# Ulixes-8/Motion-Planning-and-Control-for-Dual-Manipulator-Robot

Measured on AMD Instinct MI355X. Metric: grasp-pose IK solves/sec (Nextage dual-arm) at 1/2/4/8 MI355X, higher is better.
Workload: dtype f64

## Files before the change

motion-planning-and-control-for-dual-manipulator-robot_amd/csrc/ikg_device.hpp:

```cpp
#pragma once

#ifndef __HIPCC_RTC__
#include <hip/hip_runtime.h>
#endif
#include <stdint.h>

#include <type_traits>

#define IKG_HD __host__ __device__

#ifndef IKG_ABL
#define IKG_ABL 0
#endif
#ifndef IKG_THETA
#define IKG_THETA 0
#endif
#ifndef IKG_TAYLOR_MUL
#define IKG_TAYLOR_MUL 1
#endif
#ifndef IKG_LOG6_SERIES
#define IKG_LOG6_SERIES 1
#endif
#ifndef IKG_LANE_LIMITS
#define IKG_LANE_LIMITS 1
// ... 77 lines not shown
  static constexpr bool zero_t(int k, int i) { return (ZMASK >> (3 * k + i)) & 1; }
  static constexpr int zmask = ZMASK;
  static constexpr bool fold_hand = axis(7) != kAxRuntime && axis(7) == axis(6);
};
using SpecGeneric = Spec<kPatternGeneric, true, false>;
using SpecGenericWrist = Spec<kPatternGeneric, true, true>;
constexpr int kPatternNextage = 2 | (2 << 2) | (1 << 4) | (1 << 6) | (0 << 8) | (1 << 10) | (2 << 12) | (2 << 14);
constexpr int kZeroNextage = (3 << 3) | (1 << 6) | (2 << 9) | (6 << 12) | (3 << 15);
using SpecNextage = Spec<kPatternNextage, false, true, kZeroNextage>;

template <typename T>
struct KParams {
  T eps;
  T dt;
  T lambda;
  int32_t max_iters;
  T eps2;
};

typedef float v2f __attribute__((ext_vector_type(2)));
typedef int v2i __attribute__((ext_vector_type(2)));

template <typename T>
struct LaneT {
  using E = T;
  using M = bool;
  static constexpr bool packed = false;
};
template <>
struct LaneT<v2f> {
  using E = float;
  using M = v2i;
  static constexpr bool packed = true;
};
template <typename T>
constexpr bool is_f64 = std::is_same<typename LaneT<T>::E, double>::value;
template <typename T>
constexpr bool is_packed = LaneT<T>::packed;

IKG_HD inline bool any_of(bool m) { return m; }
IKG_HD inline bool any_of(v2i m) { return m.x != 0 || m.y != 0; }
IKG_HD inline bool all_of(bool m) { return m; }
IKG_HD inline bool all_of(v2i m) { return m.x != 0 && m.y != 0; }
#ifndef IKG_UNIFORM
#define IKG_UNIFORM 1
#endif
template <typename T>
IKG_HD inline bool wave_any(bool b) {
#if defined(__HIP_DEVICE_COMPILE__) && IKG_UNIFORM
  if constexpr (!LaneT<T>::packed) return __builtin_amdgcn_ballot_w64(b) != 0;
#endif
  return b;
}
IKG_HD inline bool mnot(bool m) { return !m; }
IKG_HD inline v2i mnot(v2i m) { return m == 0; }
IKG_HD inline bool mor(bool a, bool b) { return a || b; }
IKG_HD inline v2i mor(v2i a, v2i b) { return a | b; }
template <typename T, typename M>
IKG_HD inline T vsel(M m, T a, T b) {
  if constexpr (LaneT<T>::packed)
    return T{m.x ? a.x : b.x, m.y ? a.y : b.y};
  else
    return m ? a : b;
}

template <typename T, typename E>
IKG_HD inline T armc(bool right, E left_v, E right_v) {
  if constexpr (is_packed<T>)
    return T{left_v, right_v};
  else
    return right ? right_v : left_v;
}

using ::atan2;
using ::atan2f;
using ::fabs;
using ::fmax;
using ::fmin;
using ::sqrt;
IKG_HD inline v2f fmax(v2f a, v2f b) { return v2f{::fmaxf(a.x, b.x), ::fmaxf(a.y, b.y)}; }
IKG_HD inline v2f fmin(v2f a, v2f b) { return v2f{::fminf(a.x, b.x), ::fminf(a.y, b.y)}; }
IKG_HD inline v2f fabs(v2f a) { return v2f{::fabsf(a.x), ::fabsf(a.y)}; }
IKG_HD inline v2f sqrt(v2f a) { return v2f{::sqrtf(a.x), ::sqrtf(a.y)}; }
IKG_HD inline v2f atan2(v2f y, v2f x) { return v2f{::atan2f(y.x, x.x), ::atan2f(y.y, x.y)}; }
IKG_HD inline v2f atan2f(v2f y, v2f x) { return atan2(y, x); }

#ifndef IKG_CW_SINCOS
#define IKG_CW_SINCOS 1
#endif
#ifndef IKG_CW_SINCOS_PACKED
#define IKG_CW_SINCOS_PACKED 0
#endif
template <typename T>
IKG_HD inline void cw_poly(T r, T& sr, T& cr) {
  const T r2 = r * r;
  T sp, cp;
  if constexpr (std::is_same<T, double>::value) {
    sp = T(-1.0 / 1307674368000.0);
    sp = fma(sp, r2, T(1.0 / 6227020800.0));
    sp = fma(sp, r2, T(-1.0 / 39916800.0));
    sp = fma(sp, r2, T(1.0 / 362880.0));
    sp = fma(sp, r2, T(-1.0 / 5040.0));
    sp = fma(sp, r2, T(1.0 / 120.0));
    sp = fma(sp, r2, T(-1.0 / 6.0));
    cp = T(1.0 / 20922789888000.0);
    cp = fma(cp, r2, T(-1.0 / 87178291200.0));
// ... 343 lines not shown
  T th, st, ct;
};
template <typename T>
struct ThetaInc;
template <>
struct ThetaInc<double> {
  static constexpr double kInc = 0.05;
  IKG_HD static inline double atan_small(double r) {
    const double r2 = r * r;
    return r + r * r2 * (-1.0 / 3 + r2 * (1.0 / 5 + r2 * (-1.0 / 7 + r2 * (1.0 / 9 + r2 * (-1.0 / 11)))));
  }
  static constexpr double kIncAsin = 0.035;
  IKG_HD static inline double asin_small(double y) {
    const double y2 = y * y;
    return y + y * y2 * (1.0 / 6 + y2 * (3.0 / 40 + y2 * (5.0 / 112 + y2 * (35.0 / 1152))));
  }
};
template <>
struct ThetaInc<float> {
  static constexpr float kInc = 0.05f;
  IKG_HD static inline float atan_small(float r) {
    const float r2 = r * r;
    return r + r * r2 * (-1.0f / 3 + r2 * (1.0f / 5 + r2 * (-1.0f / 7)));
  }
  static constexpr float kIncAsin = 0.035f;
  IKG_HD static inline float asin_small(float y) {
    const float y2 = y * y;
    return y + y * y2 * (1.0f / 6 + y2 * (3.0f / 40));
  }
};

#ifndef IKG_FAST_ATAN2
#define IKG_FAST_ATAN2 1
#endif
template <typename T>
IKG_HD inline T atan2_upper(T y, T x) {
  const T ax = fabs(x);
  const T mn = fmin(ax, y), mx = fmax(ax, y);
  const T a = fdiv<T>(mn, fmax(mx, T(1e-30f)));
  const T t = a * a;
  T u = T(0.0026226534973829985f);
  u = u * t + T(-0.015134125016629696f);
  u = u * t + T(0.0411243662238121f);
  u = u * t + T(-0.07366912066936493f);
  u = u * t + T(0.1057402640581131f);
  u = u * t + T(-0.1418599784374237f);
  u = u * t + T(0.19990399479866028f);
  u = u * t + T(-0.3333298861980438f);
  T r = a + (a * t) * u;
  r = vsel<T>(y > ax, T(1.57079637f) - r, r);
  return vsel<T>(x < T(0), T(3.14159274f) - r, r);
}

template <typename T>
IKG_HD inline void log6_iter(const T* R, const T* p, T* e, ThetaTrack<T>* tk = nullptr, bool resync = true) {
  using M = typename LaneT<T>::M;
  const T pi = T(Prec<T>::kPi);
  const T tr = R[0] + R[4] + R[8];
  const T sx = R[7] - R[5], sy = R[2] - R[6], sz = R[3] - R[1];
  const T ct = (tr - T(1)) * T(0.5);
  const T st = fsqrt_unit(sx * sx + sy * sy + sz * sz) * T(0.5);
  T theta = T(0);
  if constexpr (is_f64<T>) {
    bool exact = true;
    if (tk && !resync) {
      const T y = st * tk->ct - ct * tk->st;
      const T x = ct * tk->ct + st * tk->st;
#if IKG_THETA_ASIN
      exact = !(fabs(y) <= ThetaInc<T>::kIncAsin && x > T(0));
      theta = tk->th + ThetaInc<T>::asin_small(y);
#else
      exact = !(fabs(y) <= ThetaInc<T>::kInc * x);
      theta = tk->th + ThetaInc<T>::atan_small(fdiv<T>(y, fmax(x, T(1e-30))));
#endif
    }
    if (wave_any<T>(exact)) {
#if IKG_THETA == 1
      const T th_x = atan2(st, ct);
#else
      const T th_x = acos(fmin(fmax(ct, T(-1)), T(1)));
#endif
      theta = exact ? th_x : theta;
    }
    if (tk) {
      tk->th = theta;
      tk->st = st;
      tk->ct = ct;
    }
  } else {
#if IKG_FAST_ATAN2
    theta = atan2_upper(st, ct);
#else
    theta = atan2f(st, ct);
#endif
  }
  const T t2 = theta * theta;
  const T tiny = is_f64<T> ? T(1e-300) : T(1e-30f);
  const M above = theta > T(Prec<T>::kPrec3);
  const M below = theta < T(Prec<T>::kPrec3);
  const T q = frcp<T>(fmax(t2 * st, tiny));
  const T inv_t2 = st * q;
  T f;
  if constexpr (is_f64<T>)
    f = vsel<T>(above, theta * t2 * q, T(1));
  else
    f = vsel<T>(above, theta * t2 * q, T(1) + t2 * (T(1.f / 6) + t2 * T(7.f / 360)));
  const T hf = f * T(0.5);
  T w[3] = {hf * sx, hf * sy, hf * sz};
  T alpha = hf * (T(1) + ct);
  const M near_pi = theta >= pi - T(1e-2);
  if (wave_any<T>(any_of(near_pi))) {
    const T beta = fdiv<T>(t2, T(1) - ct);
    const T t0 = (R[0] - ct) * beta, t1 = (R[4] - ct) * beta, tt = (R[8] - ct) * beta;
    const T wp0 = vsel<T>(R[7] > R[5], T(1), T(-1)) * vsel<T>(t0 > T(0), sqrt(t0), T(0));
    const T wp1 = vsel<T>(R[2] > R[6], T(1), T(-1)) * vsel<T>(t1 > T(0), sqrt(t1), T(0));
    const T wp2 = vsel<T>(R[3] > R[1], T(1), T(-1)) * vsel<T>(tt > T(0), sqrt(tt), T(0));
    w[0] = vsel<T>(near_pi, wp0, w[0]);
    w[1] = vsel<T>(near_pi, wp1, w[1]);
    w[2] = vsel<T>(near_pi, wp2, w[2]);
    alpha = vsel<T>(near_pi, fdiv<T>(theta * st, T(2) * (T(1) - ct)), alpha);
  }
  T beta;
  if constexpr (is_f64<T>) {
#if IKG_LOG6_SERIES
#if IKG_TAYLOR_MUL
    const T as = T(1) - t2 * T(1.0 / 12) - (t2 * t2) * T(1.0 / 720);
    const T bs = T(1.0 / 12) + t2 * T(1.0 / 720);
#else
    const T as = T(1) - t2 / T(12) - t2 * t2 / T(720);
    const T bs = T(1) / T(12) + t2 / T(720);
#endif
    beta = vsel<T>(below, bs, (T(1) - alpha) * inv_t2);
    alpha = vsel<T>(below, as, alpha);
#else
    (void)below;
    beta = (T(1) - alpha) * inv_t2;
#endif
  } else {
    const T as = T(1) - t2 * (T(1.f / 12) + t2 * (T(1.f / 720) + t2 * T(1.f / 30240)));
    const T bs = T(1.f / 12) + t2 * (T(1.f / 720) + t2 * (T(1.f / 30240) + t2 * T(1.f / 1209600)));
    beta = vsel<T>(below, bs, (T(1) - alpha) * inv_t2);
    alpha = vsel<T>(below, as, alpha);
  }
  const T wp = w[0] * p[0] + w[1] * p[1] + w[2] * p[2];
  const T bwp = beta * wp;
  e[0] = alpha * p[0] - T(0.5) * (w[1] * p[2] - w[2] * p[1]) + bwp * w[0];
  e[1] = alpha * p[1] - T(0.5) * (w[2] * p[0] - w[0] * p[2]) + bwp * w[1];
  e[2] = alpha * p[2] - T(0.5) * (w[0] * p[1] - w[1] * p[0]) + bwp * w[2];
  e[3] = w[0];
  e[4] = w[1];
  e[5] = w[2];
}

template <typename T>
struct Trig;
#ifndef IKG_RESYNC64
#define IKG_RESYNC64 128
#endif
#ifndef IKG_GENERIC_MED
#define IKG_GENERIC_MED 2
#endif
template <>
struct Trig<double> {
  static constexpr double kIncMax = 0.025;
// ... 187 lines not shown
  }
  T ht[3], d[3];
  if constexpr (FOLD) {
#pragma unroll
    for (int i = 0; i < 3; ++i) ht[i] = armc<T>(right, m->hand_tH[0][i], m->hand_tH[1][i]);
    matvec3(R, ht, d);
#pragma unroll
    for (int i = 0; i < 3; ++i) th[i] = t[i] + d[i];
#pragma unroll
    for (int i = 0; i < 9; ++i) Rh[i] = R[i];
  } else {
#pragma unroll
    for (int i = 0; i < 3; ++i) ht[i] = armc<T>(right, m->hand_t[0][i], m->hand_t[1][i]);
    matvec3(R, ht, d);
#pragma unroll
    for (int i = 0; i < 3; ++i) th[i] = t[i] + d[i];
    constexpr int HA = SP::axis(7);
    if constexpr (HA != kAxRuntime) {
#pragma unroll
      for (int i = 0; i < 9; ++i) Rh[i] = R[i];
      rotate_axis(Rh, HA, armc<T>(right, m->hand_sc[0][0], m->hand_sc[1][0]),
                  armc<T>(right, m->hand_sc[0][1], m->hand_sc[1][1]));
    } else {
      T hR[9];
#pragma unroll
      for (int i = 0; i < 9; ++i) hR[i] = armc<T>(right, m->hand_R[0][i], m->hand_R[1][i]);
      matmul3(R, hR, Rh);
    }
  }
}

template <typename T, class SP>
IKG_HD inline void fk_arm_world(const KModel<typename LaneT<T>::E>* __restrict__ m, int arm, const T* sn, const T* cs, T* Rh, T* th) {
  T Rc[9], tc[3];
  root_frame<T, SP>(m, sn[0], cs[0], Rc, tc);
  fk_arm<T, SP, false>(m, arm, Rc, tc, sn, cs, Rh, th, nullptr, nullptr);
}

template <typename T>
IKG_HD inline void pose_error(const T* Rh, const T* th, const T* RT, const T* tT, T* e) {
  T Rm[9], d[3], pm[3];
  matmul3_tn(Rh, RT, Rm);
#pragma unroll
  for (int i = 0; i < 3; ++i) d[i] = tT[i] - th[i];
  matvec3_t(Rh, d, pm);
  if constexpr (IKG_ABL & 2) {
    e[0] = pm[0]; e[1] = pm[1]; e[2] = pm[2];
    e[3] = T(0.5) * (Rm[7] - Rm[5]); e[4] = T(0.5) * (Rm[2] - Rm[6]); e[5] = T(0.5) * (Rm[3] - Rm[1]);
  } else {
    log6(Rm, pm, e);
  }
}

template <typename T>
IKG_HD inline void pose_error_aligned(const T* Rh, const T* th, const T* RT, const T* tT, T* e,
                                      ThetaTrack<T>* tk = nullptr, bool resync = true) {
  T Rw[9], d[3];
  matmul3_nt(RT, Rh, Rw);
#pragma unroll
  for (int i = 0; i < 3; ++i) d[i] = tT[i] - th[i];
  if constexpr (IKG_ABL & 2) {
    e[0] = d[0]; e[1] = d[1]; e[2] = d[2];
    e[3] = T(0.5) * (Rw[7] - Rw[5]); e[4] = T(0.5) * (Rw[2] - Rw[6]); e[5] = T(0.5) * (Rw[3] - Rw[1]);
  } else {
    log6_iter(Rw, d, e, tk, resync);
  }
}

template <typename T>
IKG_HD inline void qr_solve6(T (&A)[6][8], T* x0, T* x1, bool* near_singular = nullptr, T tau = T(0)) {
#pragma unroll
  for (int k = 0; k < 5; ++k) {
    T n2 = T(0);
#pragma unroll
    for (int i = k; i < 6; ++i) n2 += A[i][k] * A[i][k];
    const T nrm = sqrt(n2);
    const T akk = A[k][k];
    const T alpha = akk >= T(0) ? -nrm : nrm;
    const T vk = akk - alpha;
    const T vtv = T(2) * nrm * (nrm + fabs(akk));
    const T scale = vtv > T(0) ? T(2) / vtv : T(0);
#pragma unroll
    for (int j = k + 1; j < 8; ++j) {
      T tau = vk * A[k][j];
#pragma unroll
      for (int i = k + 1; i < 6; ++i) tau += A[i][k] * A[i][j];
      const T f = tau * scale;
      A[k][j] -= f * vk;
#pragma unroll
      for (int i = k + 1; i < 6; ++i) A[i][j] -= f * A[i][k];
    }
    A[k][k] = alpha;
  }
  T dmax = T(0);
#pragma unroll
  for (int k = 0; k < 6; ++k) dmax = fmax(dmax, fabs(A[k][k]));
  const T cut = dmax * Prec<T>::kRcond;
  if (near_singular) {
    T dmin = fabs(A[0][0]);
#pragma unroll
    for (int k = 1; k < 6; ++k) dmin = fmin(dmin, fabs(A[k][k]));
    *near_singular = dmin < tau * dmax;
  }
  T rd[6];
#pragma unroll
  for (int k = 0; k < 6; ++k) rd[k] = fabs(A[k][k]) > cut ? T(1) / A[k][k] : T(0);
#pragma unroll
  for (int r = 5; r >= 0; --r) {
    T s0 = A[r][6], s1 = A[r][7];
#pragma unroll
    for (int j = r + 1; j < 6; ++j) {
      s0 -= A[r][j] * x0[j];
      s1 -= A[r][j] * x1[j];
    }
    x0[r] = s0 * rd[r];
    x1[r] = s1 * rd[r];
  }
}
// ... 96 lines not shown
    for (int j = 0; j < 7; ++j) sn[j] += d[j];
    return;
  }
  if (big) {
    trig_exact(qc, qa, sn, cs);
  } else {
#pragma unroll
    for (int j = 0; j < 7; ++j) Trig<T>::step(d[j], sn[j], cs[j]);
  }
}

template <typename T>
IKG_HD inline void add_angles(T s1, T c1, T s2, T c2, T& s, T& c) {
  s = s1 * c2 + c1 * s2;
  c = c1 * c2 - s1 * s2;
}

template <typename T>
IKG_HD inline void trig_exact_f1(const KModel<typename LaneT<T>::E>* __restrict__ m, int arm, T qc, const T* qa, T* sn,
                                 T* cs) {
  T s[7], c[7];
  trig_exact(qc, qa, s, c);
  const bool right = arm != 0;
  const T hs = armc<T>(right, m->hand_sc[0][0], m->hand_sc[1][0]);
  const T hc = armc<T>(right, m->hand_sc[0][1], m->hand_sc[1][1]);
  add_angles(s[0], c[0], s[1], c[1], sn[0], cs[0]);
  sn[1] = s[1], cs[1] = c[1];
  sn[2] = s[2], cs[2] = c[2];
  add_angles(s[2], c[2], s[3], c[3], sn[3], cs[3]);
  sn[4] = s[4], cs[4] = c[4];
  sn[5] = s[5], cs[5] = c[5];
  add_angles(s[6], c[6], hs, hc, sn[6], cs[6]);
}

template <typename T>
IKG_HD inline void trig_med_f1(const KModel<typename LaneT<T>::E>* __restrict__ m, int arm, T qc, const T* qa,
                               const T* d, bool resync, T* sn, T* cs) {
  T dmax = fabs(d[0]);
#pragma unroll
  for (int j = 1; j < 7; ++j) dmax = fmax(dmax, fabs(d[j]));
  if (resync || any_of(dmax > T(Trig<T>::kIncMax))) {
    if (!resync && all_of(mnot(dmax > T(Trig<T>::kIncMed)))) {
#pragma unroll
      for (int j = 0; j < 7; ++j) Trig<T>::step_med(d[j], sn[j], cs[j]);
    } else {
      trig_exact_f1(m, arm, qc, qa, sn, cs);
    }
  } else {
#pragma unroll
    for (int j = 0; j < 7; ++j) Trig<T>::step(d[j], sn[j], cs[j]);
  }
}

template <typename T, bool MED = false>
IKG_HD inline void trig_advance_f1(const KModel<typename LaneT<T>::E>* __restrict__ m, int arm, T qc, const T* qa,
                                   const T* q_old, bool resync, T* sn, T* cs) {
  T dj[7], d[7];
  dj[0] = qc - q_old[0];
#pragma unroll
  for (int k = 0; k < kArmDof; ++k) dj[k + 1] = qa[k] - q_old[k + 1];
  d[0] = dj[0] + dj[1];
  d[1] = dj[1];
  d[2] = dj[2];
  d[3] = dj[2] + dj[3];
  d[4] = dj[4];
  d[5] = dj[5];
  d[6] = dj[6];
  if constexpr (!MED) {
    bool big = resync;
#pragma unroll
    for (int j = 0; j < 7; ++j) big |= any_of(fabs(d[j]) > T(Trig<T>::kIncMax));
#pragma unroll
    for (int j = 0; j < 7; ++j) Trig<T>::step(d[j], sn[j], cs[j]);
    if (wave_any<T>(big)) {
      T se[7], ce[7];
      trig_exact_f1(m, arm, qc, qa, se, ce);
#pragma unroll
      for (int j = 0; j < 7; ++j) {
        sn[j] = big ? se[j] : sn[j];
        cs[j] = big ? ce[j] : cs[j];
      }
    }
    return;
  }
  trig_med_f1(m, arm, qc, qa, d, resync, sn, cs);
}

template <typename T, class SP, bool WANT_FRAMES = false, bool WORLD = WANT_FRAMES>
IKG_HD inline T arm_fk_error(const KModel<typename LaneT<T>::E>* __restrict__ m, int arm, const T* sn, const T* cs, const T* RT,
                             const T* tT, ArmState<T>& st, T (*frames)[12] = nullptr,
                             ThetaTrack<T>* tk = nullptr, bool resync = true) {
  T Rc[9], tc[3];
  root_frame<T, SP>(m, sn[0], cs[0], Rc, tc);
  if constexpr (WORLD) {
    fk_arm<T, SP, true, WANT_FRAMES>(m, arm, Rc, tc, sn, cs, st.Rh, st.th, st.ax, st.org, frames);
    pose_error_aligned(st.Rh, st.th, RT, tT, st.e, tk, resync);
  } else {
    static_assert(!WANT_FRAMES, "joint frames are produced in the world frame");
    const T I3[9] = {T(1), T(0), T(0), T(0), T(1), T(0), T(0), T(0), T(1)};
    const T Z3[3] = {T(0), T(0), T(0)};
    fk_arm<T, SP, true>(m, arm, I3, Z3, sn, cs, st.Rh, st.th, st.ax, st.org);
    T RTc[9], dT[3], tTc[3];
    matmul3_tn(Rc, RT, RTc);
#pragma unroll
    for (int i = 0; i < 3; ++i) dT[i] = tT[i] - tc[i];
    matvec3_t(Rc, dT, tTc);
    pose_error_aligned(st.Rh, st.th, RTc, tTc, st.e, tk, resync);
  }
  const T* e = st.e;
  return e[0] * e[0] + e[1] * e[1] + e[2] * e[2] + e[3] * e[3] + e[4] * e[4] + e[5] * e[5];
}

template <typename T>
IKG_HD inline void arm_system(const ArmState<T>& st, T (&A)[6][8]) {
#pragma unroll
  for (int j = 0; j < 7; ++j) {
    const int col = j == 0 ? 7 : j - 1;
    const T dx = st.th[0] - st.org[j][0], dy = st.th[1] - st.org[j][1], dz = st.th[2] - st.org[j][2];
    A[0][col] = st.ax[j][1] * dz - st.ax[j][2] * dy;
    A[1][col] = st.ax[j][2] * dx - st.ax[j][0] * dz;
    A[2][col] = st.ax[j][0] * dy - st.ax[j][1] * dx;
    A[3][col] = st.ax[j][0];
    A[4][col] = st.ax[j][1];
    A[5][col] = st.ax[j][2];
  }
#pragma unroll
  for (int r = 0; r < 6; ++r) A[r][6] = st.e[r];
// ... 101 lines not shown
  T o2[3];
  T c12, s12;
  T k[2];
  T h[3];
  T e[6];
};

template <typename T, class SP>
IKG_HD inline void fk_f1(const KModel<typename LaneT<T>::E>* __restrict__ m, int arm, const T* sn, const T* cs,
                         ArmStateF1<T>& st, T* R) {
  static_assert(kFrame1<SP>, "frame-1 path needs the Nextage joint pattern");
  const bool right = arm != 0;
  T p0[3];
#pragma unroll
  for (int i = 0; i < 3; ++i) p0[i] = SP::zero_t(0, i) ? T(0) : armc<T>(right, m->arm_t[0][0][i], m->arm_t[1][0][i]);
  st.k[0] = cs[1] * p0[0] + sn[1] * p0[1];
  st.k[1] = cs[1] * p0[1] - sn[1] * p0[0];
#pragma unroll
  for (int i = 0; i < 9; ++i) R[i] = (i % 4 == 0) ? T(1) : T(0);
  T t[3];
#pragma unroll
  for (int i = 0; i < 3; ++i) t[i] = SP::zero_t(1, i) ? T(0) : armc<T>(right, m->arm_t[0][1][i], m->arm_t[1][1][i]);
  auto offset = [&](int k) {
    T pt[3], d[3];
#pragma unroll
    for (int i = 0; i < 3; ++i) pt[i] = SP::zero_t(k, i) ? T(0) : armc<T>(right, m->arm_t[0][k][i], m->arm_t[1][k][i]);
    matvec3(R, pt, d);
#pragma unroll
    for (int i = 0; i < 3; ++i) t[i] += d[i];
  };
  rotate_axis(R, 1, sn[2], cs[2]);
  offset(2);
#pragma unroll
  for (int i = 0; i < 3; ++i) st.o2[i] = t[i];
  st.c12 = cs[3];
  st.s12 = sn[3];
  R[0] = st.c12, R[2] = st.s12, R[6] = -st.s12, R[8] = st.c12;
  offset(3);
  rotate_axis(R, 0, sn[4], cs[4]);
  offset(4);
#pragma unroll
  for (int i = 0; i < 3; ++i) st.w[i] = t[i];
  rotate_axis(R, 1, sn[5], cs[5]);
  offset(5);
  rotate_axis(R, 2, sn[6], cs[6]);
  T ht[3], d[3];
#pragma unroll
  for (int i = 0; i < 3; ++i) ht[i] = armc<T>(right, m->hand_tH[0][i], m->hand_tH[1][i]);
  matvec3(R, ht, d);
#pragma unroll
  for (int i = 0; i < 3; ++i) st.h[i] = t[i] + d[i];
}

template <typename T, class SP>
IKG_HD inline T pose_error_f1(const KModel<typename LaneT<T>::E>* __restrict__ m, int arm, const T* sn, const T* cs,
                              const T* RT, const T* tT, ArmStateF1<T>& st, const T* R, ThetaTrack<T>* tk,
                              bool resync) {
  const bool right = arm != 0;
  const T sf = sn[0], cf = cs[0];
  const T p0z = SP::zero_t(0, 2) ? T(0) : armc<T>(right, m->arm_t[0][0][2], m->arm_t[1][0][2]);
  T RT1[9], tT1[3];
#pragma unroll
  for (int c = 0; c < 3; ++c) {
    RT1[c] = cf * RT[c] + sf * RT[3 + c];
    RT1[3 + c] = cf * RT[3 + c] - sf * RT[c];
    RT1[6 + c] = RT[6 + c];
  }
  const T d0 = tT[0] - m->root_t[0], d1 = tT[1] - m->root_t[1];
  tT1[0] = cf * d0 + sf * d1 - st.k[0];
  tT1[1] = cf * d1 - sf * d0 - st.k[1];
  tT1[2] = tT[2] - m->root_t[2] - p0z;
  pose_error_aligned(R, st.h, RT1, tT1, st.e, tk, resync);
  const T* e = st.e;
  return e[0] * e[0] + e[1] * e[1] + e[2] * e[2] + e[3] * e[3] + e[4] * e[4] + e[5] * e[5];
}

template <typename T, class SP>
IKG_HD inline T arm_fk_error_f1(const KModel<typename LaneT<T>::E>* __restrict__ m, int arm, const T* sn, const T* cs,
                                const T* RT, const T* tT, ArmStateF1<T>& st, ThetaTrack<T>* tk, bool resync) {
  T R[9];
  fk_f1<T, SP>(m, arm, sn, cs, st, R);
  return pose_error_f1<T, SP>(m, arm, sn, cs, RT, tT, st, R, tk, resync);
}

template <typename T>
struct SolveF1V {
  T iP0, iD, rH, c4r;
  T v[6];
  T beta;
};

template <typename T, class SP>
IKG_HD inline void arm_solve_f1_v(const KModel<typename LaneT<T>::E>* __restrict__ m, int arm,
                                  const ArmStateF1<T>& st, const T* sn, const T* cs, SolveF1V<T>& sv) {
  const bool right = arm != 0;
  const T* w = st.w;
  T P1[3], P2[3];
#pragma unroll
  for (int i = 0; i < 3; ++i) {
    P1[i] = SP::zero_t(1, i) ? w[i] : w[i] - armc<T>(right, m->arm_t[0][1][i], m->arm_t[1][1][i]);
    P2[i] = w[i] - st.o2[i];
  }
  const T det2 = P1[0] * P2[2] - P1[2] * P2[0];
  const T dG = w[0] * det2;
  const T rG = frcp(dG);
  sv.iP0 = det2 * rG;
  sv.iD = w[0] * rG;
  T* v = sv.v;
  {
    v[0] = (w[0] + st.k[0]) * sv.iP0;
    const T r0 = w[1] * v[0] - (w[1] + st.k[1]);
    v[1] = -P2[0] * r0 * sv.iD;
    v[2] = P1[0] * r0 * sv.iD;
  }
  const T s3 = sn[4], c3 = cs[4], s4 = sn[5], c4 = cs[5];
  sv.rH = frcp(c4);
  sv.c4r = c4 * sv.rH;
  const T c12 = st.c12, s12 = st.s12;
  {
    const T z1 = -(v[1] + v[2]), z2 = T(1) - v[0];
    const T y0 = -s12 * z2, y2 = c12 * z2;
    v[5] = (c3 * y2 - s3 * z1) * sv.rH;
    v[4] = (c3 * z1 + s3 * y2) * sv.c4r;
    v[3] = y0 - s4 * v[5];
  }
  sv.beta = T(0);
#pragma unroll
  for (int k = 0; k < 6; ++k) sv.beta += v[k] * v[k];
}

template <typename T, class SP>
IKG_HD inline void arm_solve_f1_u(const KModel<typename LaneT<T>::E>* __restrict__ m, int arm,
                                  const ArmStateF1<T>& st, const T* sn, const T* cs, const SolveF1V<T>& sv, T* u,
                                  T& alpha) {
  const bool right = arm != 0;
// ... 531 lines not shown
```

motion-planning-and-control-for-dual-manipulator-robot_amd/csrc/ikg_solve.hpp:

```cpp
#pragma once
#include "ikg_device.hpp"

namespace ikg {

template <typename T>
__device__ inline void load_q(const KModel<T>* __restrict__ m, int arm, const T* __restrict__ qrow, T& qc, T* qa) {
  qc = qrow[m->root_q];
  const bool right = arm != 0;
#pragma unroll
  for (int k = 0; k < kArmDof; ++k) qa[k] = qrow[right ? m->arm_q[1][k] : m->arm_q[0][k]];
}

template <typename T>
__device__ inline void store_q(const KModel<T>* __restrict__ m, int arm, const T* __restrict__ qrow, int it, T qc,
                               const T* qa, T* __restrict__ qo) {
  const bool right = arm != 0;
  if (!right) {
    qo[m->root_q] = qc;
    for (int i = 0; i < m->n_passive; ++i) {
      const int j = m->passive_q[i];
      const T v = qrow[j];
      qo[j] = it > 0 ? clampq(v, m->lo[j], m->hi[j]) : v;
    }
  }
// ... 112 lines not shown
  do {                                                                                        \
    __builtin_amdgcn_sched_barrier(0);                                                        \
    asm volatile("s_memtime %0\n\ts_waitcnt lgkmcnt(0)" : "=s"(t)::"memory");                 \
    __builtin_amdgcn_sched_barrier(0);                                                        \
  } while (0)
#define IKG_RSTAMP(t)                                                                         \
  do {                                                                                        \
    __builtin_amdgcn_sched_barrier(0);                                                        \
    asm volatile("s_memrealtime %0\n\ts_waitcnt lgkmcnt(0)" : "=s"(t)::"memory");             \
    __builtin_amdgcn_sched_barrier(0);                                                        \
  } while (0)
#endif

template <typename T, typename E>
__device__ inline bool both_below(T x, T xo, E eps2) {
  if constexpr (is_packed<T>)
    return all_of(x < T(eps2));
  else
    return x < eps2 && xo < eps2;
}

template <typename T>
__device__ __forceinline__ T ck_get(const typename LaneT<T>::E* c, int arm, int off) {
  if constexpr (is_packed<T>)
    return T{c[off], c[kCkArm + off]};
  else
    return c[arm * kCkArm + off];
}
template <typename T, int N>
__device__ __forceinline__ void ck_put(typename LaneT<T>::E* c, int arm, int off, const T (&v)[N]) {
  using E = typename LaneT<T>::E;
  if constexpr (is_packed<T>) {
    E a[N], b[N];
#pragma unroll
    for (int k = 0; k < N; ++k) {
      a[k] = v[k].x;
      b[k] = v[k].y;
    }
    if constexpr (N == 8) {
      store_block8(c + off, a);
      store_block8(c + kCkArm + off, b);
    } else {
      store_block4(c + off, a);
      store_block4(c + kCkArm + off, b);
    }
  } else {
    if constexpr (N == 8)
      store_block8(c + arm * kCkArm + off, v);
    else
      store_block4(c + arm * kCkArm + off, v);
  }
}

template <typename T, bool DAMPED, class SP, bool MED = false, int REC = 0>
__device__ inline bool solve_pair(const KModel<typename LaneT<T>::E>* __restrict__ m,
                                  const KParams<typename LaneT<T>::E>& prm, int arm, const T* RT, const T* tT, T& qc,
                                  T* qa, int& it_out, bool& conv_out, T& nrm_out, T& other_out,
                                  const RecOut<typename LaneT<T>::E>* ro = nullptr) {
  int k0 = -1;
  using E = typename LaneT<T>::E;
  E* recp = REC ? ro->rec : nullptr;
  static_assert(!(DAMPED && is_packed<T>), "the packed layout implements lambda = 0 only");
  constexpr bool F1 = kFrame1<SP> && !DAMPED;
  static_assert(!REC || F1, "records: the frame-1 loop only");
  T sn[7], cs[7];
  int it = 0;
  ThetaTrack<T> tk{};
  T L = T(0);
  uint64_t rbits = 0;
  if constexpr (REC == 2) {
    it = ro->it_start;
    k0 = ro->k0;
    if (it == k0) {
#pragma unroll
      for (int j = 0; j < 7; ++j) {
        sn[j] = ck_get<T>(ro->ck, arm, kCkSn + j);
        cs[j] = ck_get<T>(ro->ck, arm, kCkCs + j);
      }
      if constexpr (!is_packed<T>) {
        tk.th = ck_get<T>(ro->ck, arm, kCkTk);
        tk.st = ck_get<T>(ro->ck, arm, kCkTk + 1);
        tk.ct = ck_get<T>(ro->ck, arm, kCkTk + 2);
      }
    } else {
      trig_exact_f1(m, arm, qc, qa, sn, cs);
    }
  } else if constexpr (F1) {
    trig_exact_f1(m, arm, qc, qa, sn, cs);
  } else {
    trig_exact(qc, qa, sn, cs);
  }
  bool conv = false;
  T x, xo;
#if IKG_LANE_LIMITS
  ArmLimits<T> lim;
  if constexpr (!is_packed<T>) load_limits(m, arm, lim);
  const ArmLimits<T>* limp = is_packed<T> ? nullptr : &lim;
#else
  const ArmLimits<T>* limp = nullptr;
#endif
#ifdef IKG_PAD_OPS
  T pad[8];
#pragma unroll
  for (int i = 0; i < 8; ++i) pad[i] = qc + T(i);
#endif
#ifdef IKG_STAGE_CLOCK
  unsigned long long sc_acc[5] = {0, 0, 0, 0, 0}, sc_t0 = 0, sc_t1 = 0, sc_r0, sc_r1, sc_l0, sc_l1;
  IKG_RSTAMP(sc_r0);
  IKG_STAMP(sc_l0);
#endif
  for (;;) {
#ifdef IKG_PAD_OPS
#pragma unroll
    for (int k = 0; k < IKG_PAD_OPS / 8; ++k)
#pragma unroll
      for (int i = 0; i < 8; ++i) pad[i] = pad[i] * T(0.999999) + T(1e-7);
#endif
#if IKG_UNIFORM
    if constexpr (!is_packed<T>) it = __builtin_amdgcn_readfirstlane(it);
#endif
    ThetaTrack<T>* tkp = (IKG_THETA_TRACK && is_f64<T>) ? &tk : nullptr;
    constexpr int kRs = REC ? kRsRec<T> : Trig<T>::kResync;
    const bool resync = (it % kRs) == 0;
    T dq[6], alpha, beta, s;
    if constexpr (F1) {
      ArmStateF1<T> st;
#ifdef IKG_STAGE_CLOCK
      IKG_STAMP(sc_t0);
      x = arm_fk_error_f1<T, SP>(m, arm, sn, cs, RT, tT, st, tkp, resync);
      IKG_STAMP(sc_t1);
      sc_acc[0] += sc_t1 - sc_t0;
      pinv_step_f1<T, SP, PairX, !REC>(m, arm, st, sn, cs, dq, s);
      IKG_STAMP(sc_t0);
      sc_acc[1] += sc_t0 - sc_t1;
#else
      x = arm_fk_error_f1<T, SP>(m, arm, sn, cs, RT, tT, st, tkp, resync);
      pinv_step_f1<T, SP, PairX, !REC>(m, arm, st, sn, cs, dq, s);
#endif
    } else {
    ArmState<T> st;
    x = arm_fk_error<T, SP>(m, arm, sn, cs, RT, tT, st, nullptr, tkp, resync);
    if constexpr (!DAMPED) {
      pinv_step_cf<T, SP>(st, arm, T(m->sing_tau), T(m->sing_beta), dq, s);
    } else {
      T A[6][8], ze[6], zc[6];
      arm_system(st, A);
      arm_solve_damped(A, prm.lambda, ze, zc, alpha, beta);
      s = chest_step(alpha + pair_swap(alpha), beta + pair_swap(beta));
      arm_dq_damped(A, ze, zc, s, dq);
    }
    }
    xo = pair_swap(x);
    if constexpr (REC) {
      const bool ended = it >= prm.max_iters;
      const bool pass = !ended && both_below(x, xo, prm.eps2);
      if (pass && k0 < 0) {
        k0 = it;
        conv = true;
      }
      auto put_record = [&](E* dst) {
        if constexpr (is_packed<T>) {
          float b0[8], b1[8];
          b0[0] = qc.x;
          b1[0] = pass ? 1.f : 0.f;
#pragma unroll
          for (int k = 0; k < kArmDof; ++k) {
            b0[1 + k] = qa[k].x;
            b1[1 + k] = qa[k].y;
          }
          b0[7] = x.x;
          b1[7] = x.y;
          store_block8(dst + kRecRoot, b0);
          store_block8(dst + kRecPass, b1);
        } else {
          T blk[8];
          blk[0] = arm ? (pass ? T(1) : T(0)) : qc;
#pragma unroll
          for (int k = 0; k < kArmDof; ++k) blk[1 + k] = qa[k];
          blk[7] = x;
          store_block8(dst + (arm ? kRecPass : kRecRoot), blk);
        }
      };
      if (k0 >= 0) {
        constexpr int K = kWinOf<E>;
        const int j = it - k0;
        if constexpr (REC == 2) {
          if (pass) {
            put_record(recp + (int64_t)j * ro->rl);
            rbits |= 1ull << (it & (K - 1));
          }
          if (it + 1 >= ro->it_stop) break;
        } else {
          const bool wstart = (it & (K - 1)) == 0;
          if (wstart || j == 0) {
            E* cw = ro->ck + (int64_t)(it / K) * kCkSlot;
            const T z = T(0);
            T qb[8];
            qb[0] = qc;
#pragma unroll
            for (int k = 0; k < kArmDof; ++k) qb[1 + k] = qa[k];
            qb[7] = j == 0 ? x : L;
            ck_put<T, 8>(cw, arm, kCkQ, qb);
            if (j == 0) {
              const T sb[8] = {sn[0], sn[1], sn[2], sn[3], sn[4], sn[5], sn[6], z};
              const T cb[8] = {cs[0], cs[1], cs[2], cs[3], cs[4], cs[5], cs[6], z};
              ck_put<T, 8>(cw, arm, kCkSn, sb);
              ck_put<T, 8>(cw, arm, kCkCs, cb);
              if constexpr (!is_packed<T>) {
                const T tb[4] = {tk.th, tk.st, tk.ct, z};
                ck_put<T, 4>(cw, arm, kCkTk, tb);
              }
            }
            L = z;
          }
          if (ended) {
            E* cw = ro->ck + (int64_t)(it / K + 1) * kCkSlot;
            if constexpr (is_packed<T>) {
              cw[kCkL] = L.x;
              cw[kCkArm + kCkL] = L.y;
            } else {
              cw[arm * kCkArm + kCkL] = L;
            }
            put_record(ro->ck + ck_final<E>(prm.max_iters));
          }
        }
      }
      if (ended) break;
    } else {
      if (it >= prm.max_iters) break;
      if (both_below(x, xo, prm.eps2)) {
        conv = true;
        break;
      }
    }
    T q_old[7];
    q_old[0] = qc;
#pragma unroll
    for (int k = 0; k < kArmDof; ++k) q_old[k + 1] = qa[k];
#ifdef IKG_STAGE_CLOCK
    IKG_STAMP(sc_t1);
    sc_acc[2] += sc_t1 - sc_t0;
#endif
    arm_update(m, arm, T(prm.dt), s, dq, qc, qa, limp);
#ifndef IKG_REC_NOL_ABL
    if constexpr (REC == 1) {
      T mv = fabs(qc - q_old[0]);
#pragma unroll
      for (int k = 0; k < kArmDof; ++k) mv = fmax(mv, fabs(qa[k] - q_old[k + 1]));
      L = L + mv;
    }
#endif
    ++it;
#ifdef IKG_STAGE_CLOCK
    IKG_STAMP(sc_t0);
    sc_acc[3] += sc_t0 - sc_t1;
#endif
    if constexpr (F1) {
      trig_advance_f1<T, MED>(m, arm, qc, qa, q_old, (it % (REC ? kRsRec<T> : Trig<T>::kResync)) == 0, sn, cs);
#ifdef IKG_STAGE_CLOCK
      IKG_STAMP(sc_t1);
      sc_acc[4] += sc_t1 - sc_t0;
#endif
    } else
      trig_advance<T, MED ? 1 : IKG_GENERIC_MED>(qc, qa, q_old, (it % Trig<T>::kResync) == 0, sn, cs);
  }
#ifdef IKG_STAGE_CLOCK
  IKG_STAMP(sc_l1);
  IKG_RSTAMP(sc_r1);
  if (threadIdx.x == 0) {
    atomicAdd(&g_stage[0], 1ull);
    atomicAdd(&g_stage[1], (unsigned long long)it);
    atomicAdd(&g_stage[2], sc_l1 - sc_l0);
    atomicAdd(&g_stage[3], sc_r1 - sc_r0);
#pragma unroll
    for (int k = 0; k < 5; ++k) atomicAdd(&g_stage[4 + k], sc_acc[k]);
  }
#endif
#ifdef IKG_PAD_OPS
  T ps = T(0);
#pragma unroll
  for (int i = 0; i < 8; ++i) ps += pad[i];
  if (any_of(ps == T(-12345.678))) it = -1;
#endif
  if constexpr (REC) {
    if constexpr (REC == 2) {
      if (is_packed<T> || arm == 0) *ro->rmask = rbits;
      return true;
    }
    if (k0 >= 0) {
      const E* c0 = ro->ck + (int64_t)(k0 / kWinOf<E>) * kCkSlot;
      if constexpr (is_packed<T>) {
        float b[2][8], qa0[kArmDof];
        load_block8(c0 + kCkQ, b[0]);
        load_block8(c0 + kCkArm + kCkQ, b[1]);
#pragma unroll
        for (int h = 0; h < 2; ++h) {
#pragma unroll
          for (int k = 0; k < kArmDof; ++k) qa0[k] = b[h][1 + k];
          store_q(m, h, ro->qrow, k0, b[0][0], qa0, ro->qo);
          ro->err[h] = sqrtf(b[h][7]);
        }
        *ro->conv = 1;
        *ro->iters = k0;
        *ro->nrec = (it - k0 + 1) | kTrajEnded;
      } else {
      T blk[8];
      load_block8(c0 + arm * kCkArm + kCkQ, blk);
      T qa0[kArmDof];
#pragma unroll
      for (int k = 0; k < kArmDof; ++k) qa0[k] = blk[1 + k];
      store_q(m, arm, ro->qrow, k0, blk[0], qa0, ro->qo);
      ro->err[arm] = sqrt(blk[7]);
      if (arm == 0) {
        *ro->conv = 1;
        *ro->iters = k0;
        *ro->nrec = (it - k0 + 1) | kTrajEnded;
      }
      }
    }
  }
  it_out = it;
  nrm_out = sqrt(x);
  other_out = sqrt(xo);
  conv_out = conv;
  return REC && k0 >= 0;
}

template <typename T, bool DAMPED, class SP, bool MED, int REC = 0>
__device__ inline void pair_batch_body(const KModel<T>* __restrict__ m, const KParams<T>& prm,
                                       const T* __restrict__ targets, const T* __restrict__ q0, int64_t q0_stride,
                                       int64_t B, int64_t S, int ppw, T* __restrict__ q_out,
                                       uint8_t* __restrict__ conv_out, int32_t* __restrict__ iters_out,
                                       T* __restrict__ err_out, const RecArgs<T>& ra = RecArgs<T>{}) {
  const int lane = threadIdx.x;
  const int arm = lane & 1;
  if constexpr (REC == 2) {
    constexpr int K = kWinOf<T>;
    const int nw = rec_windows<T>(prm.max_iters);
    const int64_t n = max((int64_t)0, min((int64_t)*ra.count - ra.rbase, ra.rcap)), npad = (n + ppw - 1) / ppw * ppw;
    const int64_t wavesA = (int64_t)nw * (npad / ppw), waves = wavesA + n;
    const int rl = rec_len(m->n_passive);
    const int64_t ckpp = ck_per_problem<T>(prm.max_iters);
    for (int64_t wv = blockIdx.x; wv < waves; wv += gridDim.x) {
      int64_t i;
      int w = -1;
      if (wv < wavesA) {
        w = (int)(wv / (npad / ppw));
        i = (wv - (int64_t)w * (npad / ppw)) * ppw + (lane >> 1);
        if (lane >= 2 * ppw || i >= n) continue;
      } else {
        i = wv - wavesA;
        if (lane >= 2) continue;
      }
      const int64_t p = ra.list[ra.rbase + i];
      const int k0 = iters_out[p];
      if (w < 0) w = k0 / K;
      else if (w <= k0 / K) continue;
      if (!win_flagged(ra.wmask + p * mask_words<T>(prm.max_iters), w)) continue;
      const int64_t tgt = S > 1 ? p / S : p;
      const int64_t row = S > 1 ? p - tgt * S : p;
      T RT[9], tT[3];
      hook_target(m, arm, targets + tgt * 12, RT, tT);
      T* ckw = ra.ck + p * ckpp + (int64_t)w * kCkSlot;
      const T* cq = ckw + arm * kCkArm + kCkQ;
      T qc = cq[0], qa[kArmDof];
#pragma unroll
      for (int k = 0; k < kArmDof; ++k) qa[k] = cq[1 + k];
      RecOut<T> ro{ra.rec + i * (int64_t)(prm.max_iters + 1) * rl, ra.nrec + p, q0 + row * q0_stride,
                   q_out + p * m->nq, conv_out + p, iters_out + p, err_out + p * 2, rl, ckw};
      ro.rmask = ra.rmask + p * nw + w;
      ro.k0 = k0;
      ro.it_start = max(k0, w * K);
      ro.it_stop = min((w + 1) * K, prm.max_iters + 1);
      int it;
      bool conv;
      T nrm, other;
      solve_pair<T, DAMPED, SP, MED, 2>(m, prm, arm, RT, tT, qc, qa, it, conv, nrm, other, &ro);
    }
    return;
  }
  const int64_t p = (int64_t)blockIdx.x * ppw + (lane >> 1);
  if (lane >= 2 * ppw || p >= B) return;
  const int64_t tgt = S > 1 ? p / S : p;
  const int64_t row = S > 1 ? p - tgt * S : p;
  T RT[9], tT[3];
  hook_target(m, arm, targets + tgt * 12, RT, tT);
  const T* qrow = q0 + row * q0_stride;
  T qc, qa[kArmDof];
  load_q(m, arm, qrow, qc, qa);
  int it;
  bool conv;
  T nrm, other;
  if constexpr (REC == 1) {
    const int rl = rec_len(m->n_passive);
    RecOut<T> ro{ra.rec + p * (int64_t)(prm.max_iters + 1) * rl, ra.nrec + p, qrow, q_out + p * m->nq,
                 conv_out + p, iters_out + p, err_out + p * 2, rl, ra.ck + p * ck_per_problem<T>(prm.max_iters)};
    if (arm == 0) ra.nrec[p] = 0;
    if (solve_pair<T, DAMPED, SP, MED, 1>(m, prm, arm, RT, tT, qc, qa, it, conv, nrm, other, &ro)) return;
  } else {
    solve_pair<T, DAMPED, SP, MED>(m, prm, arm, RT, tT, qc, qa, it, conv, nrm, other);
  }
  store_q(m, arm, qrow, it, qc, qa, q_out + p * m->nq);
  if (arm == 0) {
    if (conv_out) conv_out[p] = conv ? 1 : 0;
    if (iters_out) iters_out[p] = it;
  }
  if (err_out) err_out[p * 2 + arm] = nrm;
}

}
```

Baseline: 1.645 million.

## Retire converged lanes via wave ballots and mark rare branches cold

In the scalar wave-uniform frame-1 path, lanes whose arm pair has converged write their results in-loop as soon as their ballot bits are set. The loop keeps running until every live lane is done, replacing the per-pair convergence exit and the modulo-based resync with a tracked phase. Rare branches (exact theta recompute, near-pi log, large trig steps) get __builtin_expect hints so the compiler lays them out as cold code. The aim is to cut divergence and exit bookkeeping, at the cost of converged lanes idling until the whole wave finishes, plus several padding/probe macros that are off by default.

```diff
diff --git a/motion-planning-and-control-for-dual-manipulator-robot_amd/csrc/ikg_device.hpp b/motion-planning-and-control-for-dual-manipulator-robot_amd/csrc/ikg_device.hpp
--- a/motion-planning-and-control-for-dual-manipulator-robot_amd/csrc/ikg_device.hpp
+++ b/motion-planning-and-control-for-dual-manipulator-robot_amd/csrc/ikg_device.hpp
@@ -153,6 +153,7 @@
 #endif
   return b;
 }
+#define IKG_RARELY(COLD, c) ((COLD) ? __builtin_expect((c), false) : (c))
 IKG_HD inline bool mnot(bool m) { return !m; }
 IKG_HD inline v2i mnot(v2i m) { return m == 0; }
 IKG_HD inline bool mor(bool a, bool b) { return a || b; }
@@ -602,7 +603,7 @@
   return vsel<T>(x < T(0), T(3.14159274f) - r, r);
 }
 
-template <typename T>
+template <typename T, bool COLD = false>
 IKG_HD inline void log6_iter(const T* R, const T* p, T* e, ThetaTrack<T>* tk = nullptr, bool resync = true) {
   using M = typename LaneT<T>::M;
   const T pi = T(Prec<T>::kPi);
@@ -613,7 +614,7 @@
   T theta = T(0);
   if constexpr (is_f64<T>) {
     bool exact = true;
-    if (tk && !resync) {
+    if (tk && (COLD ? __builtin_expect(!resync, true) : !resync)) {
       const T y = st * tk->ct - ct * tk->st;
       const T x = ct * tk->ct + st * tk->st;
 #if IKG_THETA_ASIN
@@ -624,7 +625,7 @@
       theta = tk->th + ThetaInc<T>::atan_small(fdiv<T>(y, fmax(x, T(1e-30))));
 #endif
     }
-    if (wave_any<T>(exact)) {
+    if (IKG_RARELY(COLD, wave_any<T>(exact))) {
 #if IKG_THETA == 1
       const T th_x = atan2(st, ct);
 #else
@@ -659,7 +660,7 @@
   T w[3] = {hf * sx, hf * sy, hf * sz};
   T alpha = hf * (T(1) + ct);
   const M near_pi = theta >= pi - T(1e-2);
-  if (wave_any<T>(any_of(near_pi))) {
+  if (IKG_RARELY(COLD, wave_any<T>(any_of(near_pi)))) {
     const T beta = fdiv<T>(t2, T(1) - ct);
     const T t0 = (R[0] - ct) * beta, t1 = (R[4] - ct) * beta, tt = (R[8] - ct) * beta;
     const T wp0 = vsel<T>(R[7] > R[5], T(1), T(-1)) * vsel<T>(t0 > T(0), sqrt(t0), T(0));
@@ -953,7 +954,7 @@
   }
 }
 
-template <typename T>
+template <typename T, bool COLD = false>
 IKG_HD inline void pose_error_aligned(const T* Rh, const T* th, const T* RT, const T* tT, T* e,
                                       ThetaTrack<T>* tk = nullptr, bool resync = true) {
   T Rw[9], d[3];
@@ -964,7 +965,7 @@
     e[0] = d[0]; e[1] = d[1]; e[2] = d[2];
     e[3] = T(0.5) * (Rw[7] - Rw[5]); e[4] = T(0.5) * (Rw[2] - Rw[6]); e[5] = T(0.5) * (Rw[3] - Rw[1]);
   } else {
-    log6_iter(Rw, d, e, tk, resync);
+    log6_iter<T, COLD>(Rw, d, e, tk, resync);
   }
 }
 
@@ -1167,7 +1168,7 @@
   }
 }
 
-template <typename T, bool MED = false>
+template <typename T, bool MED = false, bool COLD = false>
 IKG_HD inline void trig_advance_f1(const KModel<typename LaneT<T>::E>* __restrict__ m, int arm, T qc, const T* qa,
                                    const T* q_old, bool resync, T* sn, T* cs) {
   T dj[7], d[7];
@@ -1187,7 +1188,7 @@
     for (int j = 0; j < 7; ++j) big |= any_of(fabs(d[j]) > T(Trig<T>::kIncMax));
 #pragma unroll
     for (int j = 0; j < 7; ++j) Trig<T>::step(d[j], sn[j], cs[j]);
-    if (wave_any<T>(big)) {
+    if (IKG_RARELY(COLD, wave_any<T>(big))) {
       T se[7], ce[7];
       trig_exact_f1(m, arm, qc, qa, se, ce);
 #pragma unroll
@@ -1395,7 +1396,7 @@
   for (int i = 0; i < 3; ++i) st.h[i] = t[i] + d[i];
 }
 
-template <typename T, class SP>
+template <typename T, class SP, bool COLD = false>
 IKG_HD inline T pose_error_f1(const KModel<typename LaneT<T>::E>* __restrict__ m, int arm, const T* sn, const T* cs,
                               const T* RT, const T* tT, ArmStateF1<T>& st, const T* R, ThetaTrack<T>* tk,
                               bool resync) {
@@ -1413,17 +1414,17 @@
   tT1[0] = cf * d0 + sf * d1 - st.k[0];
   tT1[1] = cf * d1 - sf * d0 - st.k[1];
   tT1[2] = tT[2] - m->root_t[2] - p0z;
-  pose_error_aligned(R, st.h, RT1, tT1, st.e, tk, resync);
+  pose_error_aligned<T, COLD>(R, st.h, RT1, tT1, st.e, tk, resync);
   const T* e = st.e;
   return e[0] * e[0] + e[1] * e[1] + e[2] * e[2] + e[3] * e[3] + e[4] * e[4] + e[5] * e[5];
 }
 
-template <typename T, class SP>
+template <typename T, class SP, bool COLD = false>
 IKG_HD inline T arm_fk_error_f1(const KModel<typename LaneT<T>::E>* __restrict__ m, int arm, const T* sn, const T* cs,
                                 const T* RT, const T* tT, ArmStateF1<T>& st, ThetaTrack<T>* tk, bool resync) {
   T R[9];
   fk_f1<T, SP>(m, arm, sn, cs, st, R);
-  return pose_error_f1<T, SP>(m, arm, sn, cs, RT, tT, st, R, tk, resync);
+  return pose_error_f1<T, SP, COLD>(m, arm, sn, cs, RT, tT, st, R, tk, resync);
 }
 
 template <typename T>
diff --git a/motion-planning-and-control-for-dual-manipulator-robot_amd/csrc/ikg_solve.hpp b/motion-planning-and-control-for-dual-manipulator-robot_amd/csrc/ikg_solve.hpp
--- a/motion-planning-and-control-for-dual-manipulator-robot_amd/csrc/ikg_solve.hpp
+++ b/motion-planning-and-control-for-dual-manipulator-robot_amd/csrc/ikg_solve.hpp
@@ -188,17 +188,42 @@
   }
 }
 
+template <typename E>
+struct PassOut {
+  const E* qrow;
+  E* qo;
+  uint8_t* conv;
+  int32_t* iters;
+  E* err;
+};
+
+#ifndef IKG_SCALAR_RETIRE
+#define IKG_SCALAR_RETIRE 1
+#endif
+#ifndef IKG_COLD_PATHS
+#define IKG_COLD_PATHS 1
+#endif
+template <typename T, bool DAMPED, class SP, int REC>
+constexpr bool kScalarRetire = IKG_SCALAR_RETIRE && IKG_UNIFORM && !REC && kFrame1<SP> && !DAMPED && !is_packed<T>;
+
 template <typename T, bool DAMPED, class SP, bool MED = false, int REC = 0>
 __device__ inline bool solve_pair(const KModel<typename LaneT<T>::E>* __restrict__ m,
                                   const KParams<typename LaneT<T>::E>& prm, int arm, const T* RT, const T* tT, T& qc,
                                   T* qa, int& it_out, bool& conv_out, T& nrm_out, T& other_out,
-                                  const RecOut<typename LaneT<T>::E>* ro = nullptr) {
+                                  const RecOut<typename LaneT<T>::E>* ro = nullptr,
+                                  const PassOut<typename LaneT<T>::E>* po = nullptr) {
   int k0 = -1;
   using E = typename LaneT<T>::E;
   E* recp = REC ? ro->rec : nullptr;
   static_assert(!(DAMPED && is_packed<T>), "the packed layout implements lambda = 0 only");
   constexpr bool F1 = kFrame1<SP> && !DAMPED;
   static_assert(!REC || F1, "records: the frame-1 loop only");
+  constexpr bool RETIRE = kScalarRetire<T, DAMPED, SP, REC>;
+  constexpr bool COLD = RETIRE && IKG_COLD_PATHS;
+  uint64_t done = 0, live = 0;
+  if constexpr (RETIRE) live = __builtin_amdgcn_ballot_w64(true);
+  int stop_at = prm.max_iters;
+  int rs_phase = 0;
   T sn[7], cs[7];
   int it = 0;
   ThetaTrack<T> tk{};
@@ -240,6 +265,9 @@
 #pragma unroll
   for (int i = 0; i < 8; ++i) pad[i] = qc + T(i);
 #endif
+#ifdef IKG_PAD_SALU
+  uint32_t spad = __builtin_amdgcn_readfirstlane(prm.max_iters);
+#endif
 #ifdef IKG_STAGE_CLOCK
   unsigned long long sc_acc[5] = {0, 0, 0, 0, 0}, sc_t0 = 0, sc_t1 = 0, sc_r0, sc_r1, sc_l0, sc_l1;
   IKG_RSTAMP(sc_r0);
@@ -252,25 +280,41 @@
 #pragma unroll
       for (int i = 0; i < 8; ++i) pad[i] = pad[i] * T(0.999999) + T(1e-7);
 #endif
+#ifdef IKG_PAD_SALU
+#pragma unroll
+    for (int k = 0; k < IKG_PAD_SALU; ++k) spad = (k & 1) ? spad ^ (uint32_t)it : spad + 0x9e3779b9u;
+#endif
+#ifdef IKG_PAD_BRN
+#pragma unroll
+    for (int k = 0; k < IKG_PAD_BRN; ++k) asm volatile("s_cbranch_execz .Likg_brn%=\n.Likg_brn%=:" ::);
+#endif
+#ifdef IKG_PAD_BRT
+#pragma unroll
+    for (int k = 0; k < IKG_PAD_BRT; ++k)
+      asm volatile(
+          "s_cbranch_execnz .Likg_brt%=\n"
+          ".rept 16\n\ts_nop 0\n.endr\n"
+          ".Likg_brt%=:" ::);
+#endif
 #if IKG_UNIFORM
     if constexpr (!is_packed<T>) it = __builtin_amdgcn_readfirstlane(it);
 #endif
     ThetaTrack<T>* tkp = (IKG_THETA_TRACK && is_f64<T>) ? &tk : nullptr;
     constexpr int kRs = REC ? kRsRec<T> : Trig<T>::kResync;
-    const bool resync = (it % kRs) == 0;
+    const bool resync = RETIRE ? rs_phase == 0 : (it % kRs) == 0;
     T dq[6], alpha, beta, s;
     if constexpr (F1) {
       ArmStateF1<T> st;
 #ifdef IKG_STAGE_CLOCK
       IKG_STAMP(sc_t0);
-      x = arm_fk_error_f1<T, SP>(m, arm, sn, cs, RT, tT, st, tkp, resync);
+      x = arm_fk_error_f1<T, SP, COLD>(m, arm, sn, cs, RT, tT, st, tkp, resync);
       IKG_STAMP(sc_t1);
       sc_acc[0] += sc_t1 - sc_t0;
       pinv_step_f1<T, SP, PairX, !REC>(m, arm, st, sn, cs, dq, s);
       IKG_STAMP(sc_t0);
       sc_acc[1] += sc_t0 - sc_t1;
 #else
-      x = arm_fk_error_f1<T, SP>(m, arm, sn, cs, RT, tT, st, tkp, resync);
+      x = arm_fk_error_f1<T, SP, COLD>(m, arm, sn, cs, RT, tT, st, tkp, resync);
       pinv_step_f1<T, SP, PairX, !REC>(m, arm, st, sn, cs, dq, s);
 #endif
     } else {
@@ -362,6 +406,22 @@
         }
       }
       if (ended) break;
+    } else if constexpr (RETIRE) {
+      if (__builtin_expect(it >= stop_at, 0)) break;
+      const uint64_t fresh =
+          __builtin_amdgcn_ballot_w64(x < prm.eps2) & __builtin_amdgcn_ballot_w64(xo < prm.eps2) & ~done;
+      if (__builtin_expect(fresh != 0, 0)) {
+        if ((fresh >> (threadIdx.x & 63)) & 1) {
+          store_q(m, arm, po->qrow, it, qc, qa, po->qo);
+          if (arm == 0) {
+            if (po->conv) *po->conv = 1;
+            if (po->iters) *po->iters = it;
+          }
+          if (po->err) po->err[arm] = sqrt(x);
+        }
+        done |= fresh;
+        if (done == live) stop_at = it;
+      }
     } else {
       if (it >= prm.max_iters) break;
       if (both_below(x, xo, prm.eps2)) {
@@ -392,7 +452,9 @@
     sc_acc[3] += sc_t0 - sc_t1;
 #endif
     if constexpr (F1) {
-      trig_advance_f1<T, MED>(m, arm, qc, qa, q_old, (it % (REC ? kRsRec<T> : Trig<T>::kResync)) == 0, sn, cs);
+      if constexpr (RETIRE) rs_phase = it % Trig<T>::kResync;
+      const bool rs = RETIRE ? rs_phase == 0 : (it % (REC ? kRsRec<T> : Trig<T>::kResync)) == 0;
+      trig_advance_f1<T, MED, COLD>(m, arm, qc, qa, q_old, rs, sn, cs);
 #ifdef IKG_STAGE_CLOCK
       IKG_STAMP(sc_t1);
       sc_acc[4] += sc_t1 - sc_t0;
@@ -417,6 +479,9 @@
 #pragma unroll
   for (int i = 0; i < 8; ++i) ps += pad[i];
   if (any_of(ps == T(-12345.678))) it = -1;
+#endif
+#ifdef IKG_PAD_SALU
+  if (spad == 0x7ffffff1u) it = -1;
 #endif
   if constexpr (REC) {
     if constexpr (REC == 2) {
@@ -459,6 +524,7 @@
   nrm_out = sqrt(x);
   other_out = sqrt(xo);
   conv_out = conv;
+  if constexpr (RETIRE) return (done >> (threadIdx.x & 63)) & 1;
   return REC && k0 >= 0;
 }
 
@@ -533,6 +599,10 @@
                  conv_out + p, iters_out + p, err_out + p * 2, rl, ra.ck + p * ck_per_problem<T>(prm.max_iters)};
     if (arm == 0) ra.nrec[p] = 0;
     if (solve_pair<T, DAMPED, SP, MED, 1>(m, prm, arm, RT, tT, qc, qa, it, conv, nrm, other, &ro)) return;
+  } else if constexpr (kScalarRetire<T, DAMPED, SP, REC>) {
+    const PassOut<T> po{qrow, q_out + p * m->nq, conv_out ? conv_out + p : nullptr,
+                        iters_out ? iters_out + p : nullptr, err_out ? err_out + p * 2 : nullptr};
+    if (solve_pair<T, DAMPED, SP, MED>(m, prm, arm, RT, tT, qc, qa, it, conv, nrm, other, nullptr, &po)) return;
   } else {
     solve_pair<T, DAMPED, SP, MED>(m, prm, arm, RT, tT, qc, qa, it, conv, nrm, other);
   }
```

Measured after the change: 1.721 million, median of 6. 4.6% higher.
